# pengsongyou/openscene

Hardware: AMD Instinct MI355X
Metric: active voxels/sec MinkUNet18A fwd+bwd @2cm ScanNet; per-point query ms (higher is better)
Workload: dtype f32 (bf16x6 split-precision MFMA, fp32 accumulate); 1 GPU; ScanNet distillation step (configs[2]): MinkUNet18A, 768-d head, 1 synthetic S100k scene/GPU (100999 voxels on rank 0, 2 cm), training-mode BN; timed = coordinate+kernel maps, forward, cosine loss, backward, gradient all-reduce, Adam step; arch=MinkUNet18A, feature_dim=768, voxels_rank0=100999, parallelism=dp1

## Files before the change

### include/openscene_amd.h

```cpp
#ifndef OPENSCENE_AMD_H
#define OPENSCENE_AMD_H

#include <stddef.h>
#include <stdint.h>

#ifdef __cplusplus
extern "C" {
#endif

#define OSN_OK 0
#define OSN_E_ARG (-1)
#define OSN_E_HIP (-2)
#define OSN_E_WS (-3)
#define OSN_E_RANGE (-4)

typedef void* osn_stream_t;

int osn_version(void);
const char* osn_last_error(void);
int osn_device_ok(void);

int64_t osn_hash_capacity(int64_t n);
size_t osn_coords_unique_ws_bytes(int64_t n);

// ... 97 lines not shown
int osn_spconv_wgrad_plan(const int64_t* counts, int64_t n_out, int K, int cin, int cout,
                          int32_t* items , osn_stream_t stream);
int osn_spconv_wgrad(const float* in, const float* gout, const int32_t* nbr, const int64_t* counts,
                     const int32_t* plan_items, float* gW, int64_t n_out, int K, int cin, int cout,
                     void* ws, size_t ws_bytes, osn_stream_t stream);

size_t osn_pair_lists_bytes(int64_t n_out, int K, int bm);
int osn_pair_lists_build(const void* tl, const int32_t* out_rows, int64_t n_out, int K, int bm, void* pl,
                         osn_stream_t stream);
size_t osn_spconv_wgrad_tl_ws_bytes(int K, int cin, int cout);
int osn_spconv_wgrad_tl(const float* in, const float* gout, const void* pl, int swap, float* gW, int64_t n_in,
                        int64_t n_out, int K, int cin, int cout, void* ws, size_t ws_bytes, osn_stream_t stream);

typedef struct osn_wgrad_job {
    const float* partial;
    const void* range;
    float* gW;
    int32_t K, cin, cout, ident_items;
} osn_wgrad_job;
int osn_spconv_wgrad_tl_partial(const float* in, const float* gout, const void* pl, int swap, float* gW, int64_t n_in,
                                int64_t n_out, int K, int cin, int cout, void* partial, size_t partial_bytes,
                                osn_wgrad_job* job_host, osn_stream_t stream);
int osn_wgrad_tl_reduce_batch(const osn_wgrad_job* jobs_host, int n_jobs, osn_stream_t stream);

int osn_spconv_wgrad_tl_pieces(const float* in, const float* gout, const void* pl, int swap, float* gW, int64_t n_in,
                               int64_t n_out, int K, int cin, int cout, void* ws, size_t ws_bytes, osn_stream_t stream,
                               int pieces);
int osn_spconv_wgrad_tl_partial_pieces(const float* in, const float* gout, const void* pl, int swap, float* gW, int64_t n_in,
                                       int64_t n_out, int K, int cin, int cout, void* partial, size_t partial_bytes,
                                       osn_wgrad_job* job_host, osn_stream_t stream, int pieces);

int osn_dense_fwd(const float* in, const void* Wp, float* out, int64_t n, int cin, int cout, osn_stream_t stream);

int osn_spconv_fwd_rg_ok(int64_t n_in, int K, int cin, int cout);
int osn_spconv_fwd_rg(const float* in, int64_t n_in, const void* Wp, const int32_t* nbr, const int32_t* out_rows, float* out,
                      int64_t n_out, int K, int cin, int cout, osn_stream_t stream);

size_t osn_spconv_fwd_ws_ws_bytes(int64_t n_dst, int K, int cout, int direct);
int osn_spconv_fwd_ws(const float* in, int64_t n_in, const void* Wp, const void* pl, int64_t pl_rows, int swap, int direct,
                      const int32_t* nbr_dst, float* out, int64_t n_dst, int K, int cin, int cout, void* ws,
                      size_t ws_bytes, osn_stream_t stream);

int osn_stem_conv_fwd(const float* in, const float* W, const int32_t* nbr, float* out, int64_t n_out, int K,
                      int cin, int cout, osn_stream_t stream);
size_t osn_stem_conv_wgrad_ws_bytes(int K, int cin);
int osn_stem_conv_wgrad(const float* in, const float* gout, const int32_t* nbr, float* gW, int64_t n_out, int K, int cin,
// ... 381 lines not shown
```

### openscene_amd/_lib.py

```python
import ctypes
import os
import threading

_HERE = os.path.dirname(os.path.abspath(__file__))
LIB_PATH = os.environ.get("OSN_LIB_PATH") or os.path.join(_HERE, "lib", "libopenscene_amd.so")

_c = ctypes
_vp, _i32, _i64, _sz, _f32 = _c.c_void_p, _c.c_int, _c.c_int64, _c.c_size_t, _c.c_float

PROTOTYPES = {
    "osn_version": (_i32, []),
    "osn_last_error": (_c.c_char_p, []),
    "osn_device_ok": (_i32, []),
    "osn_hash_capacity": (_i64, [_i64]),
    "osn_coords_unique_ws_bytes": (_sz, [_i64]),
    "osn_coords_unique": (_i32, [_vp, _i64, _i32, _vp, _vp, _i64, _vp, _vp, _vp, _c.POINTER(_i64), _vp, _sz, _vp]),
    "osn_coords_unique_async": (_i32, [_vp, _i64, _vp, _i32, _vp, _vp, _i64, _vp, _vp, _vp, _vp, _vp, _vp, _sz, _vp]),
    "osn_coords_pyramid_async": (_i32, [_vp, _i64, _vp, _i32, _vp, _vp, _i64, _vp, _vp, _vp, _vp, _vp, _sz, _vp]),
    "osn_kmap_build": (_i32, [_vp, _vp, _i64, _vp, _i64, _i32, _i32, _vp, _vp, _vp]),
    "osn_kmap_build_self": (_i32, [_vp, _vp, _i64, _vp, _i64, _i32, _i32, _vp, _vp, _vp]),
    "osn_kmap_transpose": (_i32, [_vp, _i64, _i32, _i64, _vp, _vp]),
    "osn_kmap_sort_ws_bytes": (_sz, [_i64]),
    "osn_kmap_sort": (_i32, [_vp, _i64, _i32, _vp, _vp, _vp, _vp, _vp, _sz, _vp]),
    "osn_kmap_count": (_i32, [_vp, _i64, _i32, _vp, _vp]),
# ... 31 lines not shown
    "osn_spconv_wgrad_tl_ws_bytes": (_sz, [_i32, _i32, _i32]),
    "osn_spconv_wgrad_tl": (_i32, [_vp, _vp, _vp, _i32, _vp, _i64, _i64, _i32, _i32, _i32, _vp, _sz, _vp]),
    "osn_distill_loss_state_bytes": (_sz, [_i64, _i64]),
    "osn_distill_loss_fwd": (_i32, [_vp, _vp, _vp, _i64, _i64, _i32, _i32, _vp, _vp, _sz, _vp]),
    "osn_distill_loss_bwd": (_i32, [_vp, _vp, _vp, _i64, _i64, _i32, _i32, _vp, _vp, _vp, _sz, _vp]),
    "osn_rows_gather": (_i32, [_vp, _vp, _i64, _i32, _vp, _vp]),
    "osn_rows_scatter_zero": (_i32, [_vp, _vp, _i64, _i32, _vp, _vp]),
    "osn_distill_loss_check": (_i32, [_vp, _i64, _i64, _vp]),
    "osn_stem_conv_wgrad_ws_bytes": (_sz, [_i32, _i32]),
    "osn_stem_conv_wgrad": (_i32, [_vp, _vp, _vp, _vp, _i64, _i32, _i32, _i32, _vp, _sz, _vp]),
    "osn_dense_fwd": (_i32, [_vp, _vp, _vp, _i64, _i32, _i32, _vp]),
    "osn_rows_argmax": (_i32, [_vp, _i64, _i32, _vp, _i64, _i64, _vp, _vp]),
    "osn_adam_step": (_i32, [_vp, _vp, _vp, _vp, _i64, _i64, _f32, _f32, _f32, _f32, _f32, _vp]),
    "osn_sgd_step": (_i32, [_vp, _vp, _vp, _i64, _f32, _f32, _f32, _f32, _i32, _i32, _vp]),
    "osn_seg_loss_state_bytes": (_sz, [_i64, _i32]),
    "osn_seg_loss_fwd": (_i32, [_vp, _vp, _vp, _i64, _i64, _i32, _i64, _vp, _vp, _vp, _vp, _sz, _vp]),
    "osn_seg_loss_bwd": (_i32, [_vp, _vp, _vp, _i64, _i32, _i64, _vp, _vp, _sz, _vp]),
    "osn_seg_loss_check": (_i32, [_vp, _i64, _i64, _i32, _vp]),
    "osn_seg_vote": (_i32, [_vp, _vp, _i64, _i64, _i32, _vp, _vp]),
    "osn_spconv_fwd_ws_ws_bytes": (_sz, [_i64, _i32, _i32, _i32]),
    "osn_spconv_fwd_ws": (_i32, [_vp, _i64, _vp, _vp, _i64, _i32, _i32, _vp, _vp, _i64, _i32, _i32, _i32, _vp, _sz, _vp]),
    "osn_spconv_wgrad_tl_partial": (_i32, [_vp, _vp, _vp, _i32, _vp, _i64, _i64, _i32, _i32, _i32, _vp, _sz, _vp, _vp]),
    "osn_wgrad_tl_reduce_batch": (_i32, [_vp, _i32, _vp]),
    "osn_spconv_wgrad_tl_pieces": (_i32, [_vp, _vp, _vp, _i32, _vp, _i64, _i64, _i32, _i32, _i32, _vp, _sz, _vp, _i32]),
    "osn_spconv_wgrad_tl_partial_pieces": (_i32, [_vp, _vp, _vp, _i32, _vp, _i64, _i64, _i32, _i32, _i32, _vp, _sz, _vp, _vp, _i32]),
    "osn_stem_conv_fwd": (_i32, [_vp, _vp, _vp, _vp, _i64, _i32, _i32, _i32, _vp]),
    "osn_bn_ws_bytes": (_sz, [_i64, _i32]),
    "osn_bn_stats": (_i32, [_vp, _i64, _i32, _vp, _vp, _vp, _vp, _f32, _vp, _sz, _vp]),
    "osn_bn_apply": (_i32, [_vp, _vp, _vp, _vp, _vp, _f32, _vp, _i32, _vp, _vp, _i64, _i64, _i32, _vp]),
    "osn_spconv_fwd_rg_ok": (_i32, [_i64, _i32, _i32, _i32]),
    "osn_spconv_fwd_rg": (_i32, [_vp, _i64, _vp, _vp, _vp, _vp, _i64, _i32, _i32, _i32, _vp]),
    "osn_bn_forward_train": (_i32, [_vp, _i64, _i32, _vp, _vp, _f32, _vp, _i32, _f32, _vp, _vp, _vp, _vp, _vp, _vp, _i64, _vp, _sz, _vp]),
    "osn_bn_backward": (_i32, [_vp, _vp, _vp, _vp, _i32, _vp, _vp, _vp, _vp, _f32, _i32, _i32, _vp, _vp, _vp, _vp, _i64, _i32,
                               _vp, _sz, _vp]),
    "osn_bn_apply_plan": (_i32, [_i64, _i32, _c.POINTER(_i32), _c.POINTER(_i32)]),
    "osn_bn_set_flat_kernels": (_i32, [_i32]),
    "osn_bn_set_separate_finalize": (_i32, [_i32]),
    "osn_net_plan_query": (_i32, [_vp, _vp, _i32, _vp]),
    "osn_net_forward": (_i32, [_vp, _vp, _vp]),
    "osn_net_backward": (_i32, [_vp, _vp, _vp]),
    "osn_maps_build": (_i32, [_vp, _i32, _vp, _i32, _vp, _vp, _vp, _i32, _vp]),
    "osn_maps_occupancy_bytes": (_sz, [_i64]),
    "osn_maps_build_occ": (_i32, [_vp, _i32, _vp, _i32, _vp, _vp, _vp, _i32, _vp, _vp]),
    "osn_maps_set_legacy": (_i32, [_i32]),
    "osn_events_create": (_vp, [_i32]),
    "osn_events_destroy": (None, [_vp]),
# ... 139 lines not shown
```

### openscene_amd/csrc/pairlist.h

```cpp
#pragma once
#include "common.h"

namespace osn {

constexpr int PL_KMAX = 128;
constexpr int PL_ITEMS = 512;
constexpr int PL_MIN_QUOTA = 256;

constexpr size_t PL_OFF_POFF = 0;
constexpr size_t PL_OFF_TOTAL = 1024;
constexpr size_t PL_OFF_ITEMS = 2048;
constexpr size_t PL_OFF_RANGE = PL_OFF_ITEMS + size_t(PL_ITEMS) * 16;
constexpr size_t PL_OFF_PAIRS = 16384;

struct PlView {
    int32_t *poff, *total;
    int4* items;
    int2* range;
    int32_t *pin, *pout, *pref;
    size_t bytes;
};

static PlView pl_view(void* base, int64_t n_out, int K, int bm) {
    PlView v;
    char* p = static_cast<char*>(base);
    const size_t cap = size_t(K) * size_t(n_out > 0 ? n_out : 1);
    const size_t nt = size_t(cdiv(n_out > 0 ? n_out : 1, bm > 0 ? bm : 1));
    v.poff = reinterpret_cast<int32_t*>(p + PL_OFF_POFF);
    v.total = reinterpret_cast<int32_t*>(p + PL_OFF_TOTAL);
    v.items = reinterpret_cast<int4*>(p + PL_OFF_ITEMS);
// ... 10 lines not shown
```

### openscene_amd/csrc/wgrad_tl.hip

```cpp
#include "common.h"
#include "split.h"
#include <cstdlib>
#include "pairlist.h"
#include "coords_impl.h"

namespace osn {

typedef short s16x4 __attribute__((ext_vector_type(4)));

__device__ inline int wave_incl_scan_i32(int v, int lane) {
#pragma unroll
    for (int d = 1; d < 64; d <<= 1) {
        const int t = __shfl_up(v, d, 64);
        if (lane >= d) v += t;
    }
    return v;
}

__global__ __launch_bounds__(256) void pair_prefix_kernel(const int32_t* __restrict__ cnt, int n_tiles, int K,
                                                          int32_t* __restrict__ pref, int32_t* __restrict__ total) {
    __shared__ int wtot[4];
    __shared__ int carry_s;
    const int k = blockIdx.x, tid = threadIdx.x, lane = tid & 63, wave = tid >> 6;
    if (tid == 0) carry_s = 0;
// ... 83 lines not shown
    if (tid < K) range[tid] = make_int2(start[tid], start[tid + 1]);
    for (int t = tid; t < PL_ITEMS; t += 256) {
        int4 it = make_int4(-1, 0, 0, 0);
        if (t < start[K]) {
            int k = 0;
            while (k + 1 < K && start[k + 1] <= t) ++k;
            const int j = t - start[k];
            it.x = k;
            it.y = j * quota;
            it.z = min(it.y + quota, total[k]);
        }
        items[t] = it;
    }
}

__global__ __launch_bounds__(256) void pair_plan_kernel(const int32_t* __restrict__ total, int K, int4* __restrict__ items,
                                                        int2* __restrict__ range, int items_max) {
    pair_plan(total, K, items, range, items_max);
}

#define OSN_WG_TEMPLATE template <int MB, int NB, bool BUFG = false>
#define OSN_WG_NAME wgrad_tl_kernel
#define OSN_WG_NP 3
#include "wgrad_tl_kernel.h"
#undef OSN_WG_TEMPLATE
#undef OSN_WG_NAME
#undef OSN_WG_NP
#define OSN_WG_TEMPLATE template <int NP_, int MB, int NB, bool BUFG = false>
#define OSN_WG_NAME wgrad_tl_pieces_kernel
#define OSN_WG_NP NP_
#include "wgrad_tl_kernel.h"
#undef OSN_WG_TEMPLATE
#undef OSN_WG_NAME
#undef OSN_WG_NP

__global__ void wgrad_tl_reduce_kernel(const float* __restrict__ partial, const int2* __restrict__ range, int K, int cin,
                                       int cout, int transpose, int ident_items, float* __restrict__ out) {
    const int64_t per_k = int64_t(cin) * cout;
    const int64_t total = int64_t(K) * per_k;
    for (int64_t e = int64_t(blockIdx.x) * blockDim.x + threadIdx.x; e < total; e += int64_t(gridDim.x) * blockDim.x) {
        const int k = int(e / per_k);
        const int64_t r = e - int64_t(k) * per_k;
        int64_t src = r;
        if (transpose) {
            const int ci = int(r / cout), co = int(r - int64_t(ci) * cout);
            src = int64_t(co) * cin + ci;
        }
        const int t0 = range ? range[k].x : 0, t1 = range ? range[k].y : ident_items;
        float s = 0.f;
        for (int t = t0; t < t1; ++t) s += partial[int64_t(t) * per_k + src];
        out[e] = s;
    }
}

constexpr int WG_BATCH = 32;
struct WgJobs {
    osn_wgrad_job j[WG_BATCH];
};
// ... 51 lines not shown
        OSN_HIP(hipMemsetAsync(v.items, 0xFF, size_t(PL_ITEMS) * 16, st));
        OSN_HIP(hipMemsetAsync(v.range, 0, size_t(PL_KMAX) * 8, st));
        return OSN_OK;
    }
    OSN_REQUIRE(tl, OSN_E_ARG, "osn_pair_lists_build: null tile lists");
    const int64_t nt = cdiv(n_out, bm);
    const int32_t* cnt = static_cast<const int32_t*>(tl);
    const int2* lst = reinterpret_cast<const int2*>(static_cast<const char*>(tl) + align_up(size_t(nt) * K * 4, 256));
    hipLaunchKernelGGL(pair_prefix_kernel, dim3(K), dim3(256), 0, st, cnt, int(nt), K, v.pref, v.total);
    const int items_max = PL_ITEMS;
    const bool own_plan = maps_legacy();
    if (own_plan) hipLaunchKernelGGL(pair_plan_kernel, dim3(1), dim3(256), 0, st, v.total, K, v.items, v.range, items_max);
    hipLaunchKernelGGL(pair_fill_kernel, dim3(unsigned(nt)), dim3(256), 0, st, cnt, lst, out_rows, v.pref, v.total, int(nt), K,
                       bm, v.pin, v.pout, v.poff, own_plan ? nullptr : v.items, v.range, items_max);
    OSN_LAUNCH_CHECK();
    return OSN_OK;
}

namespace {
struct WgTlPlan {
    int mb, nb, n_ab, n_gb;
};
WgTlPlan plan_wg_tl(int ca, int cg) {
    auto blocks = [](int c) { int t = (c + 31) / 32; return t > 4 ? 4 : t; };
    WgTlPlan p;
    p.mb = blocks(ca);
    p.nb = blocks(cg);
    p.n_ab = int(cdiv(ca, 32 * p.mb));
    p.n_gb = int(cdiv(cg, 32 * p.nb));
    return p;
}
int ident_quota(int64_t n) {
    int64_t q = cdiv(n, PL_ITEMS);
    q = (q + 31) / 32 * 32;
    if (q < 64) q = 64;
    return int(q);
}
}

extern "C" size_t osn_spconv_wgrad_tl_ws_bytes(int K, int cin, int cout) {
    (void)K;
    return size_t(PL_ITEMS) * size_t(cin) * size_t(cout) * 4;
}

template <int MB>
static void launch_wg_tl_nb(int pieces, int nb, dim3 grid, hipStream_t st, const float* ra, const float* rg, const int32_t* ia,
                            const int32_t* ig, const int32_t* poff, const int4* items, float* partial, int ca, int cg,
                            int n_gb, int irows, int iquota, unsigned a_bytes, unsigned g_bytes) {
    const bool bufg = a_bytes != 0u && g_bytes != 0u;
#define OSN_WGTL_L(...)                                                                                                        \
    do {                                                                                                                       \
        if (bufg)                                                                                                              \
            hipLaunchKernelGGL((__VA_ARGS__, true>), grid, dim3(256), 0, st, ra, rg, ia, ig, poff, items, partial, ca, cg, n_gb, irows, \
                               iquota, a_bytes, g_bytes);                                                                      \
        else                                                                                                                   \
            hipLaunchKernelGGL((__VA_ARGS__, false>), grid, dim3(256), 0, st, ra, rg, ia, ig, poff, items, partial, ca, cg, n_gb, irows, \
                               iquota, 0u, 0u);                                                                                \
    } while (0)
#define OSN_WGTL(NB_)                                                                                                          \
    do {                                                                                                                       \
        if (pieces == 3) OSN_WGTL_L(wgrad_tl_kernel<MB, NB_);                                                                  \
        else if (pieces == 2) OSN_WGTL_L(wgrad_tl_pieces_kernel<2, MB, NB_);                                                   \
        else OSN_WGTL_L(wgrad_tl_pieces_kernel<1, MB, NB_);                                                                    \
    } while (0)
    switch (nb) {
        case 1: OSN_WGTL(1); break;
        case 2: OSN_WGTL(2); break;
        case 3: OSN_WGTL(3); break;
        default: OSN_WGTL(4); break;
    }
#undef OSN_WGTL
#undef OSN_WGTL_L
}

static int wgrad_tl_partial(const float* in, const float* gout, const void* pl, int swap, float* gW, int64_t n_in,
                            int64_t n_out, int K, int cin, int cout, void* ws, size_t ws_bytes, osn_wgrad_job* job,
                            int* launched, osn_stream_t stream, int pieces) {
    hipStream_t st = static_cast<hipStream_t>(stream);
    OSN_REQUIRE(pieces >= 1 && pieces <= 3, OSN_E_ARG, "osn_spconv_wgrad_tl: pieces=%d (1, 2 or 3)", pieces);
    OSN_REQUIRE(K >= 1 && K <= PL_KMAX && cin >= 4 && (cin & 3) == 0 && cout >= 4 && (cout & 3) == 0 && gW, OSN_E_ARG,
                "osn_spconv_wgrad_tl: needs cin %% 4 == 0 and cout %% 4 == 0 (K=%d cin=%d cout=%d)", K, cin, cout);
    OSN_REQUIRE(n_in >= 0 && n_out >= 0 && n_in < (int64_t(1) << 31) && n_out < (int64_t(1) << 31), OSN_E_ARG,
                "osn_spconv_wgrad_tl: row counts out of range");
    const int64_t wtotal = int64_t(K) * cin * cout;
    *launched = 0;
    if (n_out == 0 || n_in == 0) {
        OSN_HIP(hipMemsetAsync(gW, 0, size_t(wtotal) * 4, st));
        return OSN_OK;
    }
    OSN_REQUIRE(in && gout, OSN_E_ARG, "osn_spconv_wgrad_tl: null pointer");
    OSN_REQUIRE(pl || (K == 1 && n_in == n_out), OSN_E_ARG, "osn_spconv_wgrad_tl: pair lists may be null only for K == 1");
    OSN_REQUIRE(aligned16(in) && aligned16(gout) && aligned16(gW), OSN_E_ARG, "osn_spconv_wgrad_tl: pointers must be 16-byte aligned");
    const size_t need = osn_spconv_wgrad_tl_ws_bytes(K, cin, cout);
    OSN_REQUIRE(ws && ws_bytes >= need, OSN_E_WS, "osn_spconv_wgrad_tl: workspace %zu < %zu", ws_bytes, need);
    float* partial = static_cast<float*>(ws);
// ... 3 lines not shown
    const int32_t *ia = nullptr, *ig = nullptr, *poff = nullptr;
    const int4* items = nullptr;
    const int2* range = nullptr;
    int n_items = PL_ITEMS, irows = 0, iquota = 0;
    if (pl) {
        const int64_t table_rows = swap ? n_in : n_out;
        PlView v = pl_view(const_cast<void*>(pl), table_rows, K, 1);
        ia = swap ? v.pout : v.pin;
        ig = swap ? v.pin : v.pout;
        poff = v.poff;
        items = v.items;
        range = v.range;
    } else {
        irows = int(n_out);
        iquota = ident_quota(n_out);
        n_items = int(cdiv(n_out, iquota));
    }
    const WgTlPlan p = plan_wg_tl(ca, cg);
    const dim3 grid(unsigned(p.n_ab * p.n_gb), unsigned(n_items));
    const uint64_t ab64 = uint64_t(n_in) * uint64_t(cin) * 4u, gb64 = uint64_t(n_out) * uint64_t(cout) * 4u;
    const bool bufg = n_in < (int64_t(1) << 24) && n_out < (int64_t(1) << 24) && ab64 < (uint64_t(1) << 31) &&
                      gb64 < (uint64_t(1) << 31);
    const unsigned a_bytes = bufg ? unsigned(ab64) : 0u, g_bytes = bufg ? unsigned(gb64) : 0u;
    switch (p.mb) {
        case 1: launch_wg_tl_nb<1>(pieces, p.nb, grid, st, ra, rg, ia, ig, poff, items, partial, ca, cg, p.n_gb, irows, iquota, a_bytes, g_bytes); break;
        case 2: launch_wg_tl_nb<2>(pieces, p.nb, grid, st, ra, rg, ia, ig, poff, items, partial, ca, cg, p.n_gb, irows, iquota, a_bytes, g_bytes); break;
        case 3: launch_wg_tl_nb<3>(pieces, p.nb, grid, st, ra, rg, ia, ig, poff, items, partial, ca, cg, p.n_gb, irows, iquota, a_bytes, g_bytes); break;
        default: launch_wg_tl_nb<4>(pieces, p.nb, grid, st, ra, rg, ia, ig, poff, items, partial, ca, cg, p.n_gb, irows, iquota, a_bytes, g_bytes); break;
    }
    OSN_LAUNCH_CHECK();
    job->partial = partial;
    job->range = range;
    job->gW = gW;
    job->K = K; job->cin = cin; job->cout = cout; job->ident_items = n_items;
    *launched = 1;
    return OSN_OK;
}

static int wgrad_tl_whole(const float* in, const float* gout, const void* pl, int swap, float* gW, int64_t n_in, int64_t n_out, int K,
                          int cin, int cout, void* ws, size_t ws_bytes, osn_stream_t stream, int pieces) {
    hipStream_t st = static_cast<hipStream_t>(stream);
    osn_wgrad_job job;
    int launched = 0;
    int rc = wgrad_tl_partial(in, gout, pl, swap, gW, n_in, n_out, K, cin, cout, ws, ws_bytes, &job, &launched, stream, pieces);
    if (rc || !launched) return rc;
    const int64_t wtotal = int64_t(K) * cin * cout;
    int g = int(cdiv(wtotal, 256));
    if (g > 4096) g = 4096;
    hipLaunchKernelGGL(wgrad_tl_reduce_kernel, dim3(g), dim3(256), 0, st, job.partial, static_cast<const int2*>(job.range), K, cin,
                       cout, 0, job.ident_items, gW);
    OSN_LAUNCH_CHECK();
// ... 63 lines not shown
```

### openscene_amd/csrc/wgrad_tl_kernel.h

```cpp
OSN_WG_TEMPLATE
__global__ __launch_bounds__(256, 2) void OSN_WG_NAME(const float* __restrict__ rows_a, const float* __restrict__ rows_g,
                                                      const int32_t* __restrict__ idx_a, const int32_t* __restrict__ idx_g,
                                                      const int32_t* __restrict__ poff, const int4* __restrict__ items,
                                                      float* __restrict__ partial, int ca, int cg, int n_cgb,
                                                      int ident_rows, int ident_quota, unsigned a_bytes, unsigned g_bytes) {
    constexpr int NP = OSN_WG_NP;
    constexpr int CA_T = 32 * MB, CG_T = 32 * NB;
    constexpr int LDA = CA_T + 8, LDG = CG_T + 8;
    constexpr int QA = CA_T / 4, QG = CG_T / 4;
    __shared__ __attribute__((aligned(16))) __bf16 Ap[NP][32][LDA];
    __shared__ __attribute__((aligned(16))) __bf16 Gp[NP][32][LDG];
    __shared__ int idxbuf[2][32];

    const int tid = threadIdx.x, lane = tid & 63;
    const int wave = __builtin_amdgcn_readfirstlane(tid >> 6);
    const int wi = wave >> 1, wj = wave & 1;
    const int a0 = (blockIdx.x / n_cgb) * CA_T;
    const int g0 = (blockIdx.x % n_cgb) * CG_T;
    int k, p0, p1, base;
    int pstep = 32;
    if (idx_a) {
        const int4 it = items[blockIdx.y];
        k = it.x; p0 = it.y; p1 = it.z;
        if (k < 0) return;
        base = poff[k];
        const int n_it = it.w >> 16;
        if (n_it > 1) { p0 += 32 * (it.w & 0xFFFF); pstep = 32 * n_it; }
        if (p0 >= p1) p1 = p0;
    } else {
        k = 0; base = 0;
        p0 = blockIdx.y * ident_quota;
        p1 = min(p0 + ident_quota, ident_rows);
        if (p0 >= p1) return;
    }
    (void)k;

    f32x4 acc[MB][NB];
#pragma unroll
    for (int i = 0; i < MB; ++i)
#pragma unroll
        for (int j = 0; j < NB; ++j) acc[i][j] = f32x4{0.f, 0.f, 0.f, 0.f};

    int ar[MB], ac[MB], gr[NB], gc[NB];
#pragma unroll
    for (int j = 0; j < MB; ++j) { const int idx = tid + 256 * j; ar[j] = idx / QA; ac[j] = (idx - ar[j] * QA) * 4; }
#pragma unroll
    for (int j = 0; j < NB; ++j) { const int idx = tid + 256 * j; gr[j] = idx / QG; gc[j] = (idx - gr[j] * QG) * 4; }

    const __amdgpu_buffer_rsrc_t arsrc = __builtin_amdgcn_make_buffer_rsrc(const_cast<float*>(rows_a), 0, int(BUFG ? a_bytes : 0u), 0x00020000);
    const __amdgpu_buffer_rsrc_t grsrc = __builtin_amdgcn_make_buffer_rsrc(const_cast<float*>(rows_g), 0, int(BUFG ? g_bytes : 0u), 0x00020000);
    const unsigned ca4 = unsigned(ca) * 4u, cg4 = unsigned(cg) * 4u;
    float4 pa[MB], pg[NB];
    auto load_idx = [&](int p) -> int {
        const int q = p + (tid & 31);
        if (tid >= 64) return -1;
        if (q >= p1) return -1;
        if (!idx_a) return q;
        return tid < 32 ? idx_a[base + q] : idx_g[base + q];
    };
    auto fetch = [&](int par) {
#pragma unroll
        for (int j = 0; j < MB; ++j) {
            const int r = idxbuf[0][ar[j]];
            const int ch = a0 + ac[j];
            if constexpr (BUFG) {
                pa[j] = __builtin_bit_cast(float4, __builtin_amdgcn_raw_buffer_load_b128(
                                                       arsrc, __umul24(unsigned(max(r, 0)), ca4) + 4u * unsigned(ch), 0, 0));
                continue;
            }
            const bool ok = r >= 0 && ch < ca;
            const unsigned ru = ok ? unsigned(r) : 0u, cu = ok ? unsigned(ch) : 0u;
            pa[j] = *reinterpret_cast<const float4*>(rows_a + (uint64_t(ru) * unsigned(ca) + cu));
        }
#pragma unroll
        for (int j = 0; j < NB; ++j) {
            const int r = idxbuf[1][gr[j]];
            const int ch = g0 + gc[j];
            if constexpr (BUFG) {
                pg[j] = __builtin_bit_cast(float4, __builtin_amdgcn_raw_buffer_load_b128(
                                                       grsrc, __umul24(unsigned(max(r, 0)), cg4) + 4u * unsigned(ch), 0, 0));
                continue;
            }
            const bool ok = r >= 0 && ch < cg;
            const unsigned ru = ok ? unsigned(r) : 0u, cu = ok ? unsigned(ch) : 0u;
            pg[j] = *reinterpret_cast<const float4*>(rows_g + (uint64_t(ru) * unsigned(cg) + cu));
        }
        (void)par;
    };
    auto split4 = [&](const float4& v, bool ok, bf16x4& h1, bf16x4& h2, bf16x4& h3) {
        bf16x4 h[NP];
        tl_split4<NP>(ok ? v : make_float4(0.f, 0.f, 0.f, 0.f), h);
        h1 = h[0];
        if constexpr (NP > 1) h2 = h[1];
        if constexpr (NP > 2) h3 = h[2];
    };

    int ireg = load_idx(p0);
    if (tid < 64) idxbuf[tid >> 5][tid & 31] = ireg;
    __syncthreads();
    bool ok_a[MB], ok_g[NB];
    auto valid_now = [&]() {
#pragma unroll
        for (int j = 0; j < MB; ++j) ok_a[j] = idxbuf[0][ar[j]] >= 0 && a0 + ac[j] < ca;
#pragma unroll
        for (int j = 0; j < NB; ++j) ok_g[j] = idxbuf[1][gr[j]] >= 0 && g0 + gc[j] < cg;
    };
    valid_now();
    fetch(0);
    ireg = load_idx(p0 + pstep);

    for (int p = p0; p < p1; p += pstep) {
        bf16x4 a1[MB], a2[MB], a3[MB], g1[NB], g2[NB], g3[NB];
#pragma unroll
        for (int j = 0; j < MB; ++j) split4(pa[j], ok_a[j], a1[j], a2[j], a3[j]);
#pragma unroll
        for (int j = 0; j < NB; ++j) split4(pg[j], ok_g[j], g1[j], g2[j], g3[j]);
        __syncthreads();
#pragma unroll
        for (int j = 0; j < MB; ++j) {
            *reinterpret_cast<bf16x4*>(&Ap[0][ar[j]][ac[j]]) = a1[j];
            if constexpr (NP > 1) *reinterpret_cast<bf16x4*>(&Ap[1][ar[j]][ac[j]]) = a2[j];
            if constexpr (NP > 2) *reinterpret_cast<bf16x4*>(&Ap[2][ar[j]][ac[j]]) = a3[j];
        }
#pragma unroll
        for (int j = 0; j < NB; ++j) {
            *reinterpret_cast<bf16x4*>(&Gp[0][gr[j]][gc[j]]) = g1[j];
            if constexpr (NP > 1) *reinterpret_cast<bf16x4*>(&Gp[1][gr[j]][gc[j]]) = g2[j];
            if constexpr (NP > 2) *reinterpret_cast<bf16x4*>(&Gp[2][gr[j]][gc[j]]) = g3[j];
        }
        if (tid < 64) idxbuf[tid >> 5][tid & 31] = ireg;
        __syncthreads();
        if (p + pstep < p1) {
            valid_now();
            fetch(0);
            ireg = load_idx(p + 2 * pstep);
        }
        const int li = lane & 15, lg = lane >> 4;
        auto frag = [&](const __bf16* plane, int pitch, int c16) -> bf16x8 {
            const __bf16* q = plane + (8 * lg + (li >> 2)) * pitch + c16 + 4 * (li & 3);
            const s16x4 lo = __builtin_amdgcn_ds_read_tr16_b64_v4i16(
                (__attribute__((address_space(3))) s16x4*)(q));
            const s16x4 hi = __builtin_amdgcn_ds_read_tr16_b64_v4i16(
                (__attribute__((address_space(3))) s16x4*)(q + 4 * pitch));
            union { s16x4 h[2]; bf16x8 v; } u;
            u.h[0] = lo; u.h[1] = hi;
            return u.v;
        };
        bf16x8 fa[MB][NP], fg[NB][NP];
#pragma unroll
        for (int i = 0; i < MB; ++i)
#pragma unroll
            for (int pl = 0; pl < NP; ++pl) fa[i][pl] = frag(&Ap[pl][0][0], LDA, (wi * MB + i) * 16);
#pragma unroll
        for (int j = 0; j < NB; ++j)
#pragma unroll
            for (int pl = 0; pl < NP; ++pl) fg[j][pl] = frag(&Gp[pl][0][0], LDG, (wj * NB + j) * 16);
#pragma unroll
        for (int i = 0; i < MB; ++i)
#pragma unroll
            for (int j = 0; j < NB; ++j) {
                f32x4 t = acc[i][j];
                split_products<NP>([&](auto ap, auto gp) {
                    t = __builtin_amdgcn_mfma_f32_16x16x32_bf16(fa[i][ap], fg[j][gp], t, 0, 0, 0);
                });
                acc[i][j] = t;
            }
    }

    float* d = partial + int64_t(blockIdx.y) * ca * cg;
#pragma unroll
    for (int i = 0; i < MB; ++i)
#pragma unroll
        for (int j = 0; j < NB; ++j) {
            const int co = g0 + (wj * NB + j) * 16 + (lane & 15);
#pragma unroll
            for (int r = 0; r < 4; ++r) {
                const int ci = a0 + (wi * MB + i) * 16 + 4 * (lane >> 4) + r;
                if (ci < ca && co < cg) d[int64_t(ci) * cg + co] = acc[i][j][r];
            }
        }
}
```

### openscene_amd/ops.py

```python
import ctypes
import os
import threading
import weakref

import torch

from . import _lib
from ._lib import check

_vp = ctypes.c_void_p

_profiler = None


def set_profiler(p):
    global _profiler
    _profiler = p


_raw_stream_of = torch._C._cuda_getCurrentRawStream
_current_device = torch._C._cuda_getDevice


def _prof_start(kind, dev, **meta):
# ... 631 lines not shown
    if tl is not None:
        table_rows = n_in if swap else n_out
        if tl.K != K or tl.n_out != table_rows:
            raise ValueError("pair lists are for a [%d, %d] table, the weight gradient wants [%d, %d]" % (
                tl.K, tl.n_out, K, table_rows))
        pl = pair_lists(tl)
    else:
        if K != 1 or n_in != n_out:
            raise ValueError("tl=None is the identity map and needs K == 1 and n_in == n_out")
        pl = None
    gw = torch.empty((K, cin, cout), dtype=torch.float32, device=dev)
    wsb = _cached("osn_spconv_wgrad_tl_ws_bytes", K, cin, cout)
    ws = _ws(wsb, dev)
    tok = _prof_start("spconv_wgrad_tl", dev, n_in=n_in, n_out=n_out, K=K, cin=cin, cout=cout)
    with _Dev(dev):
        args = (_p(feats), _p(gout), _p(pl), int(bool(swap)), _p(gw), n_in, n_out, K, cin, cout, _p(ws), ws.numel(), _stream(dev))
        if pieces == 3:
            check(lib.osn_spconv_wgrad_tl(*args), "osn_spconv_wgrad_tl")
        else:
            check(lib.osn_spconv_wgrad_tl_pieces(*args, pieces), "osn_spconv_wgrad_tl_pieces")
    if tok is not None:
        _profiler.stop(tok)
    return gw


def rows_argmax(scores, gather=None):
    dev = scores.device
    lib = _prep(dev)
    if scores.dtype != torch.float32 or scores.dim() != 2 or scores.stride(1) != 1:
        raise ValueError("scores must be a float32 matrix with unit column stride")
    n, c = scores.shape
    ld = scores.stride(0) if n > 1 else max(c, scores.stride(0))
    if gather is not None:
        if gather.dtype != torch.int64 or gather.device != dev:
            raise ValueError("gather must be an int64 vector on the scores' device")
        gather = gather.contiguous()
    n_pts = n if gather is None else gather.shape[0]
    labels = torch.empty(n_pts, dtype=torch.int64, device=dev)
    with _Dev(dev):
        check(lib.osn_rows_argmax(_p(scores), ld, c, _p(gather), n_pts, n, _p(labels), _stream(dev)), "osn_rows_argmax")
    return labels


def dense_eligible(cin, cout):
    return bool(_cached("osn_dense_fwd_ok", int(cin), int(cout)))

# ... 1982 lines not shown
```

Before: 13.23 million voxels/s.

## Process multiple 32-pair sub-steps per iteration in narrow wgrad tiles

The weight-gradient pair-list kernel now stages several 32-pair sub-tiles (64 or 128 pairs) in LDS per loop iteration for narrow channel tiles (MB,NB<=2), picked by a constexpr table by tile shape and split pieces. Each barrier pair and index load then covers more MFMA work, which cuts sync overhead and exposes more memory-level parallelism for small-channel layers. It adds a runtime override (atomic global plus C API) that dispatches to extra template instantiations. The cost is higher LDS and register use, which can lower occupancy, and more padded work at segment tails.

Measured after the change: 13.23 million voxels/s (median of 3 runs). Within noise of the previous version (+0.0%).

```diff
diff --git a/include/openscene_amd.h b/include/openscene_amd.h
--- a/include/openscene_amd.h
+++ b/include/openscene_amd.h
@@ -143,6 +143,9 @@
                                 int64_t n_out, int K, int cin, int cout, void* partial, size_t partial_bytes,
                                 osn_wgrad_job* job_host, osn_stream_t stream);
 int osn_wgrad_tl_reduce_batch(const osn_wgrad_job* jobs_host, int n_jobs, osn_stream_t stream);
+
+int osn_spconv_wgrad_tl_step_pairs(int cin, int cout, int pieces);
+int osn_wgrad_tl_set_step_pairs(int pairs);
 
 int osn_spconv_wgrad_tl_pieces(const float* in, const float* gout, const void* pl, int swap, float* gW, int64_t n_in,
                                int64_t n_out, int K, int cin, int cout, void* ws, size_t ws_bytes, osn_stream_t stream,
diff --git a/openscene_amd/_lib.py b/openscene_amd/_lib.py
--- a/openscene_amd/_lib.py
+++ b/openscene_amd/_lib.py
@@ -77,6 +77,8 @@
     "osn_spconv_fwd_ws": (_i32, [_vp, _i64, _vp, _vp, _i64, _i32, _i32, _vp, _vp, _i64, _i32, _i32, _i32, _vp, _sz, _vp]),
     "osn_spconv_wgrad_tl_partial": (_i32, [_vp, _vp, _vp, _i32, _vp, _i64, _i64, _i32, _i32, _i32, _vp, _sz, _vp, _vp]),
     "osn_wgrad_tl_reduce_batch": (_i32, [_vp, _i32, _vp]),
+    "osn_spconv_wgrad_tl_step_pairs": (_i32, [_i32, _i32, _i32]),
+    "osn_wgrad_tl_set_step_pairs": (_i32, [_i32]),
     "osn_spconv_wgrad_tl_pieces": (_i32, [_vp, _vp, _vp, _i32, _vp, _i64, _i64, _i32, _i32, _i32, _vp, _sz, _vp, _i32]),
     "osn_spconv_wgrad_tl_partial_pieces": (_i32, [_vp, _vp, _vp, _i32, _vp, _i64, _i64, _i32, _i32, _i32, _vp, _sz, _vp, _vp, _i32]),
     "osn_stem_conv_fwd": (_i32, [_vp, _vp, _vp, _vp, _i64, _i32, _i32, _i32, _vp]),
diff --git a/openscene_amd/csrc/pairlist.h b/openscene_amd/csrc/pairlist.h
--- a/openscene_amd/csrc/pairlist.h
+++ b/openscene_amd/csrc/pairlist.h
@@ -6,6 +6,19 @@
 constexpr int PL_KMAX = 128;
 constexpr int PL_ITEMS = 512;
 constexpr int PL_MIN_QUOTA = 256;
+
+constexpr int tl_wg_blocks(int c) { return (c + 31) / 32 > 4 ? 4 : (c + 31) / 32; }
+constexpr int tl_step_lds(int mb, int nb, int np, int ps) { return np * ps * ((32 * mb + 8) + (32 * nb + 8)) * 2 + 8 * ps; }
+constexpr bool tl_step_narrow(int mb, int nb) { return mb <= 2 && nb <= 2; }
+constexpr int tl_step_pairs_blocks(int mb, int nb, int np) {
+    if (!tl_step_narrow(mb, nb)) return 32;
+    if (mb == 1 && nb == 1) return np == 3 ? 32 : 128;
+    if (mb == 1 && nb == 2) return 64;
+    if (mb == 2 && nb == 1) return np == 1 ? 32 : 64;
+    return 32;
+}
+static_assert(tl_step_lds(1, 1, 2, 128) <= 65536 && tl_step_lds(1, 2, 3, 64) <= 65536 && tl_step_lds(2, 1, 3, 64) <= 65536, "LDS budget");
+constexpr int tl_step_pairs(int cin, int cout, int pieces) { return tl_step_pairs_blocks(tl_wg_blocks(cin), tl_wg_blocks(cout), pieces); }
 
 constexpr size_t PL_OFF_POFF = 0;
 constexpr size_t PL_OFF_TOTAL = 1024;
diff --git a/openscene_amd/csrc/wgrad_tl.hip b/openscene_amd/csrc/wgrad_tl.hip
--- a/openscene_amd/csrc/wgrad_tl.hip
+++ b/openscene_amd/csrc/wgrad_tl.hip
@@ -1,5 +1,6 @@
 #include "common.h"
 #include "split.h"
+#include <atomic>
 #include <cstdlib>
 #include "pairlist.h"
 #include "coords_impl.h"
@@ -129,18 +130,21 @@
 #define OSN_WG_TEMPLATE template <int MB, int NB, bool BUFG = false>
 #define OSN_WG_NAME wgrad_tl_kernel
 #define OSN_WG_NP 3
+#define OSN_WG_PS tl_step_pairs_blocks(MB, NB, 3)
 #include "wgrad_tl_kernel.h"
 #undef OSN_WG_TEMPLATE
 #undef OSN_WG_NAME
 #undef OSN_WG_NP
-#define OSN_WG_TEMPLATE template <int NP_, int MB, int NB, bool BUFG = false>
+#undef OSN_WG_PS
+#define OSN_WG_TEMPLATE template <int NP_, int MB, int NB, bool BUFG = false, int PS_ = 0>
 #define OSN_WG_NAME wgrad_tl_pieces_kernel
 #define OSN_WG_NP NP_
+#define OSN_WG_PS (PS_ ? PS_ : tl_step_pairs_blocks(MB, NB, NP_))
 #include "wgrad_tl_kernel.h"
 #undef OSN_WG_TEMPLATE
 #undef OSN_WG_NAME
 #undef OSN_WG_NP
-
+#undef OSN_WG_PS
 __global__ void wgrad_tl_reduce_kernel(const float* __restrict__ partial, const int2* __restrict__ range, int K, int cin,
                                        int cout, int transpose, int ident_items, float* __restrict__ out) {
     const int64_t per_k = int64_t(cin) * cout;
@@ -238,10 +242,9 @@
     int mb, nb, n_ab, n_gb;
 };
 WgTlPlan plan_wg_tl(int ca, int cg) {
-    auto blocks = [](int c) { int t = (c + 31) / 32; return t > 4 ? 4 : t; };
     WgTlPlan p;
-    p.mb = blocks(ca);
-    p.nb = blocks(cg);
+    p.mb = tl_wg_blocks(ca);
+    p.nb = tl_wg_blocks(cg);
     p.n_ab = int(cdiv(ca, 32 * p.mb));
     p.n_gb = int(cdiv(cg, 32 * p.nb));
     return p;
@@ -259,34 +262,79 @@
     return size_t(PL_ITEMS) * size_t(cin) * size_t(cout) * 4;
 }
 
+static std::atomic<int> g_step_pairs{0};
+
+namespace {
+struct WgTlLaunch {
+    dim3 grid;
+    hipStream_t st;
+    const float *ra, *rg;
+    const int32_t *ia, *ig, *poff;
+    const int4* items;
+    float* partial;
+    int ca, cg, n_gb, irows, iquota;
+    unsigned a_bytes, g_bytes;
+};
+template <typename Kernel>
+void launch_wg_tl(Kernel kern, const WgTlLaunch& a) {
+    hipLaunchKernelGGL(kern, a.grid, dim3(256), 0, a.st, a.ra, a.rg, a.ia, a.ig, a.poff, a.items, a.partial, a.ca, a.cg, a.n_gb, a.irows,
+                       a.iquota, a.a_bytes, a.g_bytes);
+}
+template <int PS, int NP, int MB, int NB>
+void launch_wg_tl_step(bool bufg, const WgTlLaunch& a) {
+    if constexpr (tl_step_lds(MB, NB, NP, PS) <= 65536 && PS != tl_step_pairs_blocks(MB, NB, NP)) {
+        if (bufg) launch_wg_tl(wgrad_tl_pieces_kernel<NP, MB, NB, true, PS>, a);
+        else launch_wg_tl(wgrad_tl_pieces_kernel<NP, MB, NB, false, PS>, a);
+    }
+}
+template <int NP, int MB, int NB>
+void launch_wg_tl_inst(const WgTlLaunch& a) {
+    const bool bufg = a.a_bytes != 0u && a.g_bytes != 0u;
+    if constexpr (tl_step_narrow(MB, NB)) {
+        int want = g_step_pairs.load(std::memory_order_relaxed);
+        while (want > 32 && tl_step_lds(MB, NB, NP, want) > 65536) want /= 2;
+        if (want != 0 && want != tl_step_pairs_blocks(MB, NB, NP)) {
+            if (want == 128) launch_wg_tl_step<128, NP, MB, NB>(bufg, a);
+            else if (want == 64) launch_wg_tl_step<64, NP, MB, NB>(bufg, a);
+            else launch_wg_tl_step<32, NP, MB, NB>(bufg, a);
+            return;
+        }
+    }
+    if constexpr (NP == 3) {
+        if (bufg) launch_wg_tl(wgrad_tl_kernel<MB, NB, true>, a);
+        else launch_wg_tl(wgrad_tl_kernel<MB, NB, false>, a);
+    } else {
+        if (bufg) launch_wg_tl(wgrad_tl_pieces_kernel<NP, MB, NB, true>, a);
+        else launch_wg_tl(wgrad_tl_pieces_kernel<NP, MB, NB, false>, a);
+    }
+}
+template <int MB, int NB>
+void launch_wg_tl_np(int pieces, const WgTlLaunch& a) {
+    if (pieces == 3) launch_wg_tl_inst<3, MB, NB>(a);
+    else if (pieces == 2) launch_wg_tl_inst<2, MB, NB>(a);
+    else launch_wg_tl_inst<1, MB, NB>(a);
+}
 template <int MB>
-static void launch_wg_tl_nb(int pieces, int nb, dim3 grid, hipStream_t st, const float* ra, const float* rg, const int32_t* ia,
-                            const int32_t* ig, const int32_t* poff, const int4* items, float* partial, int ca, int cg,
-                            int n_gb, int irows, int iquota, unsigned a_bytes, unsigned g_bytes) {
-    const bool bufg = a_bytes != 0u && g_bytes != 0u;
-#define OSN_WGTL_L(...)                                                                                                        \
-    do {                                                                                                                       \
-        if (bufg)                                                                                                              \
-            hipLaunchKernelGGL((__VA_ARGS__, true>), grid, dim3(256), 0, st, ra, rg, ia, ig, poff, items, partial, ca, cg, n_gb, irows, \
-                               iquota, a_bytes, g_bytes);                                                                      \
-        else                                                                                                                   \
-            hipLaunchKernelGGL((__VA_ARGS__, false>), grid, dim3(256), 0, st, ra, rg, ia, ig, poff, items, partial, ca, cg, n_gb, irows, \
-                               iquota, 0u, 0u);                                                                                \
-    } while (0)
-#define OSN_WGTL(NB_)                                                                                                          \
-    do {                                                                                                                       \
-        if (pieces == 3) OSN_WGTL_L(wgrad_tl_kernel<MB, NB_);                                                                  \
-        else if (pieces == 2) OSN_WGTL_L(wgrad_tl_pieces_kernel<2, MB, NB_);                                                   \
-        else OSN_WGTL_L(wgrad_tl_pieces_kernel<1, MB, NB_);                                                                    \
-    } while (0)
+void launch_wg_tl_nb(int pieces, int nb, const WgTlLaunch& a) {
     switch (nb) {
-        case 1: OSN_WGTL(1); break;
-        case 2: OSN_WGTL(2); break;
-        case 3: OSN_WGTL(3); break;
-        default: OSN_WGTL(4); break;
-    }
-#undef OSN_WGTL
-#undef OSN_WGTL_L
+        case 1: launch_wg_tl_np<MB, 1>(pieces, a); break;
+        case 2: launch_wg_tl_np<MB, 2>(pieces, a); break;
+        case 3: launch_wg_tl_np<MB, 3>(pieces, a); break;
+        default: launch_wg_tl_np<MB, 4>(pieces, a); break;
+    }
+}
+}
+
+extern "C" int osn_spconv_wgrad_tl_step_pairs(int cin, int cout, int pieces) {
+    OSN_REQUIRE(cin >= 1 && cout >= 1 && pieces >= 1 && pieces <= 3, OSN_E_ARG, "osn_spconv_wgrad_tl_step_pairs: cin=%d cout=%d pieces=%d",
+                cin, cout, pieces);
+    return tl_step_pairs(cin, cout, pieces);
+}
+
+extern "C" int osn_wgrad_tl_set_step_pairs(int pairs) {
+    OSN_REQUIRE(pairs == 0 || pairs == 32 || pairs == 64 || pairs == 128, OSN_E_ARG, "osn_wgrad_tl_set_step_pairs: %d (0, 32, 64 or 128)",
+                pairs);
+    return g_step_pairs.exchange(pairs);
 }
 
 static int wgrad_tl_partial(const float* in, const float* gout, const void* pl, int swap, float* gW, int64_t n_in,
@@ -336,11 +384,12 @@
     const bool bufg = n_in < (int64_t(1) << 24) && n_out < (int64_t(1) << 24) && ab64 < (uint64_t(1) << 31) &&
                       gb64 < (uint64_t(1) << 31);
     const unsigned a_bytes = bufg ? unsigned(ab64) : 0u, g_bytes = bufg ? unsigned(gb64) : 0u;
+    const WgTlLaunch la{grid, st, ra, rg, ia, ig, poff, items, partial, ca, cg, p.n_gb, irows, iquota, a_bytes, g_bytes};
     switch (p.mb) {
-        case 1: launch_wg_tl_nb<1>(pieces, p.nb, grid, st, ra, rg, ia, ig, poff, items, partial, ca, cg, p.n_gb, irows, iquota, a_bytes, g_bytes); break;
-        case 2: launch_wg_tl_nb<2>(pieces, p.nb, grid, st, ra, rg, ia, ig, poff, items, partial, ca, cg, p.n_gb, irows, iquota, a_bytes, g_bytes); break;
-        case 3: launch_wg_tl_nb<3>(pieces, p.nb, grid, st, ra, rg, ia, ig, poff, items, partial, ca, cg, p.n_gb, irows, iquota, a_bytes, g_bytes); break;
-        default: launch_wg_tl_nb<4>(pieces, p.nb, grid, st, ra, rg, ia, ig, poff, items, partial, ca, cg, p.n_gb, irows, iquota, a_bytes, g_bytes); break;
+        case 1: launch_wg_tl_nb<1>(pieces, p.nb, la); break;
+        case 2: launch_wg_tl_nb<2>(pieces, p.nb, la); break;
+        case 3: launch_wg_tl_nb<3>(pieces, p.nb, la); break;
+        default: launch_wg_tl_nb<4>(pieces, p.nb, la); break;
     }
     OSN_LAUNCH_CHECK();
     job->partial = partial;
diff --git a/openscene_amd/csrc/wgrad_tl_kernel.h b/openscene_amd/csrc/wgrad_tl_kernel.h
--- a/openscene_amd/csrc/wgrad_tl_kernel.h
+++ b/openscene_amd/csrc/wgrad_tl_kernel.h
@@ -8,9 +8,14 @@
     constexpr int CA_T = 32 * MB, CG_T = 32 * NB;
     constexpr int LDA = CA_T + 8, LDG = CG_T + 8;
     constexpr int QA = CA_T / 4, QG = CG_T / 4;
-    __shared__ __attribute__((aligned(16))) __bf16 Ap[NP][32][LDA];
-    __shared__ __attribute__((aligned(16))) __bf16 Gp[NP][32][LDG];
-    __shared__ int idxbuf[2][32];
+    constexpr int PS = OSN_WG_PS, NS = PS / 32;
+    static_assert(PS == 32 || PS == 64 || PS == 128, "pairs per step");
+    static_assert(tl_step_lds(MB, NB, NP, PS) <= 65536, "two workgroups per CU");
+    struct __attribute__((aligned(16))) StageA { __bf16 Ap[NP][32][LDA]; };
+    struct __attribute__((aligned(16))) StageG { __bf16 Gp[NP][32][LDG]; };
+    __shared__ StageA sa[NS];
+    __shared__ StageG sg[NS];
+    __shared__ int idxbuf[2][PS];
 
     const int tid = threadIdx.x, lane = tid & 63;
     const int wave = __builtin_amdgcn_readfirstlane(tid >> 6);
@@ -50,40 +55,47 @@
     const __amdgpu_buffer_rsrc_t arsrc = __builtin_amdgcn_make_buffer_rsrc(const_cast<float*>(rows_a), 0, int(BUFG ? a_bytes : 0u), 0x00020000);
     const __amdgpu_buffer_rsrc_t grsrc = __builtin_amdgcn_make_buffer_rsrc(const_cast<float*>(rows_g), 0, int(BUFG ? g_bytes : 0u), 0x00020000);
     const unsigned ca4 = unsigned(ca) * 4u, cg4 = unsigned(cg) * 4u;
-    float4 pa[MB], pg[NB];
+    float4 pa[NS][MB], pg[NS][NB];
+    const int isub = NS == 1 ? 0 : tid >> 6, ihalf = NS == 1 ? tid >> 5 : (tid >> 5) & 1;
     auto load_idx = [&](int p) -> int {
-        const int q = p + (tid & 31);
-        if (tid >= 64) return -1;
+        const int q = p + isub * pstep + (tid & 31);
+        if (tid >= 64 * NS) return -1;
         if (q >= p1) return -1;
         if (!idx_a) return q;
-        return tid < 32 ? idx_a[base + q] : idx_g[base + q];
+        return (NS == 1 ? tid < 32 : ihalf == 0) ? idx_a[base + q] : idx_g[base + q];
+    };
+    auto store_idx = [&](int v) {
+        if (tid < 64 * NS) idxbuf[ihalf][32 * isub + (tid & 31)] = v;
     };
     auto fetch = [&](int par) {
 #pragma unroll
-        for (int j = 0; j < MB; ++j) {
-            const int r = idxbuf[0][ar[j]];
-            const int ch = a0 + ac[j];
-            if constexpr (BUFG) {
-                pa[j] = __builtin_bit_cast(float4, __builtin_amdgcn_raw_buffer_load_b128(
-                                                       arsrc, __umul24(unsigned(max(r, 0)), ca4) + 4u * unsigned(ch), 0, 0));
-                continue;
-            }
-            const bool ok = r >= 0 && ch < ca;
-            const unsigned ru = ok ? unsigned(r) : 0u, cu = ok ? unsigned(ch) : 0u;
-            pa[j] = *reinterpret_cast<const float4*>(rows_a + (uint64_t(ru) * unsigned(ca) + cu));
-        }
-#pragma unroll
-        for (int j = 0; j < NB; ++j) {
-            const int r = idxbuf[1][gr[j]];
-            const int ch = g0 + gc[j];
-            if constexpr (BUFG) {
-                pg[j] = __builtin_bit_cast(float4, __builtin_amdgcn_raw_buffer_load_b128(
-                                                       grsrc, __umul24(unsigned(max(r, 0)), cg4) + 4u * unsigned(ch), 0, 0));
-                continue;
-            }
-            const bool ok = r >= 0 && ch < cg;
-            const unsigned ru = ok ? unsigned(r) : 0u, cu = ok ? unsigned(ch) : 0u;
-            pg[j] = *reinterpret_cast<const float4*>(rows_g + (uint64_t(ru) * unsigned(cg) + cu));
+        for (int s = 0; s < NS; ++s) {
+#pragma unroll
+            for (int j = 0; j < MB; ++j) {
+                const int r = idxbuf[0][32 * s + ar[j]];
+                const int ch = a0 + ac[j];
+                if constexpr (BUFG) {
+                    pa[s][j] = __builtin_bit_cast(float4, __builtin_amdgcn_raw_buffer_load_b128(
+                                                           arsrc, __umul24(unsigned(max(r, 0)), ca4) + 4u * unsigned(ch), 0, 0));
+                    continue;
+                }
+                const bool ok = r >= 0 && ch < ca;
+                const unsigned ru = ok ? unsigned(r) : 0u, cu = ok ? unsigned(ch) : 0u;
+                pa[s][j] = *reinterpret_cast<const float4*>(rows_a + (uint64_t(ru) * unsigned(ca) + cu));
+            }
+#pragma unroll
+            for (int j = 0; j < NB; ++j) {
+                const int r = idxbuf[1][32 * s + gr[j]];
+                const int ch = g0 + gc[j];
+                if constexpr (BUFG) {
+                    pg[s][j] = __builtin_bit_cast(float4, __builtin_amdgcn_raw_buffer_load_b128(
+                                                           grsrc, __umul24(unsigned(max(r, 0)), cg4) + 4u * unsigned(ch), 0, 0));
+                    continue;
+                }
+                const bool ok = r >= 0 && ch < cg;
+                const unsigned ru = ok ? unsigned(r) : 0u, cu = ok ? unsigned(ch) : 0u;
+                pg[s][j] = *reinterpret_cast<const float4*>(rows_g + (uint64_t(ru) * unsigned(cg) + cu));
+            }
         }
         (void)par;
     };
@@ -95,45 +107,55 @@
         if constexpr (NP > 2) h3 = h[2];
     };
 
+    const int bstep = NS * pstep;
     int ireg = load_idx(p0);
-    if (tid < 64) idxbuf[tid >> 5][tid & 31] = ireg;
+    store_idx(ireg);
     __syncthreads();
-    bool ok_a[MB], ok_g[NB];
+    bool ok_a[NS][MB], ok_g[NS][NB];
     auto valid_now = [&]() {
 #pragma unroll
-        for (int j = 0; j < MB; ++j) ok_a[j] = idxbuf[0][ar[j]] >= 0 && a0 + ac[j] < ca;
-#pragma unroll
-        for (int j = 0; j < NB; ++j) ok_g[j] = idxbuf[1][gr[j]] >= 0 && g0 + gc[j] < cg;
+        for (int s = 0; s < NS; ++s) {
+#pragma unroll
+            for (int j = 0; j < MB; ++j) ok_a[s][j] = idxbuf[0][32 * s + ar[j]] >= 0 && a0 + ac[j] < ca;
+#pragma unroll
+            for (int j = 0; j < NB; ++j) ok_g[s][j] = idxbuf[1][32 * s + gr[j]] >= 0 && g0 + gc[j] < cg;
+        }
     };
     valid_now();
     fetch(0);
-    ireg = load_idx(p0 + pstep);
-
-    for (int p = p0; p < p1; p += pstep) {
-        bf16x4 a1[MB], a2[MB], a3[MB], g1[NB], g2[NB], g3[NB];
-#pragma unroll
-        for (int j = 0; j < MB; ++j) split4(pa[j], ok_a[j], a1[j], a2[j], a3[j]);
-#pragma unroll
-        for (int j = 0; j < NB; ++j) split4(pg[j], ok_g[j], g1[j], g2[j], g3[j]);
+    ireg = load_idx(p0 + bstep);
+
+    for (int p = p0; p < p1; p += bstep) {
+        bf16x4 a1[NS][MB], a2[NS][MB], a3[NS][MB], g1[NS][NB], g2[NS][NB], g3[NS][NB];
+#pragma unroll
+        for (int s = 0; s < NS; ++s) {
+#pragma unroll
+            for (int j = 0; j < MB; ++j) split4(pa[s][j], ok_a[s][j], a1[s][j], a2[s][j], a3[s][j]);
+#pragma unroll
+            for (int j = 0; j < NB; ++j) split4(pg[s][j], ok_g[s][j], g1[s][j], g2[s][j], g3[s][j]);
+        }
         __syncthreads();
 #pragma unroll
-        for (int j = 0; j < MB; ++j) {
-            *reinterpret_cast<bf16x4*>(&Ap[0][ar[j]][ac[j]]) = a1[j];
-            if constexpr (NP > 1) *reinterpret_cast<bf16x4*>(&Ap[1][ar[j]][ac[j]]) = a2[j];
-            if constexpr (NP > 2) *reinterpret_cast<bf16x4*>(&Ap[2][ar[j]][ac[j]]) = a3[j];
-        }
-#pragma unroll
-        for (int j = 0; j < NB; ++j) {
-            *reinterpret_cast<bf16x4*>(&Gp[0][gr[j]][gc[j]]) = g1[j];
-            if constexpr (NP > 1) *reinterpret_cast<bf16x4*>(&Gp[1][gr[j]][gc[j]]) = g2[j];
-            if constexpr (NP > 2) *reinterpret_cast<bf16x4*>(&Gp[2][gr[j]][gc[j]]) = g3[j];
-        }
-        if (tid < 64) idxbuf[tid >> 5][tid & 31] = ireg;
+        for (int s = 0; s < NS; ++s) {
+#pragma unroll
+            for (int j = 0; j < MB; ++j) {
+                *reinterpret_cast<bf16x4*>(&sa[s].Ap[0][ar[j]][ac[j]]) = a1[s][j];
+                if constexpr (NP > 1) *reinterpret_cast<bf16x4*>(&sa[s].Ap[1][ar[j]][ac[j]]) = a2[s][j];
+                if constexpr (NP > 2) *reinterpret_cast<bf16x4*>(&sa[s].Ap[2][ar[j]][ac[j]]) = a3[s][j];
+            }
+#pragma unroll
+            for (int j = 0; j < NB; ++j) {
+                *reinterpret_cast<bf16x4*>(&sg[s].Gp[0][gr[j]][gc[j]]) = g1[s][j];
+                if constexpr (NP > 1) *reinterpret_cast<bf16x4*>(&sg[s].Gp[1][gr[j]][gc[j]]) = g2[s][j];
+                if constexpr (NP > 2) *reinterpret_cast<bf16x4*>(&sg[s].Gp[2][gr[j]][gc[j]]) = g3[s][j];
+            }
+        }
+        store_idx(ireg);
         __syncthreads();
-        if (p + pstep < p1) {
+        if (p + bstep < p1) {
             valid_now();
             fetch(0);
-            ireg = load_idx(p + 2 * pstep);
+            ireg = load_idx(p + 2 * bstep);
         }
         const int li = lane & 15, lg = lane >> 4;
         auto frag = [&](const __bf16* plane, int pitch, int c16) -> bf16x8 {
@@ -146,25 +168,28 @@
             u.h[0] = lo; u.h[1] = hi;
             return u.v;
         };
-        bf16x8 fa[MB][NP], fg[NB][NP];
-#pragma unroll
-        for (int i = 0; i < MB; ++i)
-#pragma unroll
-            for (int pl = 0; pl < NP; ++pl) fa[i][pl] = frag(&Ap[pl][0][0], LDA, (wi * MB + i) * 16);
-#pragma unroll
-        for (int j = 0; j < NB; ++j)
-#pragma unroll
-            for (int pl = 0; pl < NP; ++pl) fg[j][pl] = frag(&Gp[pl][0][0], LDG, (wj * NB + j) * 16);
-#pragma unroll
-        for (int i = 0; i < MB; ++i)
-#pragma unroll
-            for (int j = 0; j < NB; ++j) {
-                f32x4 t = acc[i][j];
-                split_products<NP>([&](auto ap, auto gp) {
-                    t = __builtin_amdgcn_mfma_f32_16x16x32_bf16(fa[i][ap], fg[j][gp], t, 0, 0, 0);
-                });
-                acc[i][j] = t;
-            }
+#pragma unroll
+        for (int s = 0; s < NS; ++s) {
+            bf16x8 fa[MB][NP], fg[NB][NP];
+#pragma unroll
+            for (int i = 0; i < MB; ++i)
+#pragma unroll
+                for (int pl = 0; pl < NP; ++pl) fa[i][pl] = frag(&sa[s].Ap[pl][0][0], LDA, (wi * MB + i) * 16);
+#pragma unroll
+            for (int j = 0; j < NB; ++j)
+#pragma unroll
+                for (int pl = 0; pl < NP; ++pl) fg[j][pl] = frag(&sg[s].Gp[pl][0][0], LDG, (wj * NB + j) * 16);
+#pragma unroll
+            for (int i = 0; i < MB; ++i)
+#pragma unroll
+                for (int j = 0; j < NB; ++j) {
+                    f32x4 t = acc[i][j];
+                    split_products<NP>([&](auto ap, auto gp) {
+                        t = __builtin_amdgcn_mfma_f32_16x16x32_bf16(fa[i][ap], fg[j][gp], t, 0, 0, 0);
+                    });
+                    acc[i][j] = t;
+                }
+        }
     }
 
     float* d = partial + int64_t(blockIdx.y) * ca * cg;
diff --git a/openscene_amd/ops.py b/openscene_amd/ops.py
--- a/openscene_amd/ops.py
+++ b/openscene_amd/ops.py
@@ -677,6 +677,18 @@
     if tok is not None:
         _profiler.stop(tok)
     return gw
+
+
+def wgrad_tl_step_pairs(cin, cout, pieces=3):
+    ps = int(_lib.load().osn_spconv_wgrad_tl_step_pairs(int(cin), int(cout), int(pieces)))
+    check(min(ps, 0), "osn_spconv_wgrad_tl_step_pairs")
+    return ps
+
+
+def wgrad_tl_set_step_pairs(pairs):
+    prev = int(_lib.load().osn_wgrad_tl_set_step_pairs(int(pairs)))
+    check(min(prev, 0), "osn_wgrad_tl_set_step_pairs")
+    return prev
 
 
 def rows_argmax(scores, gather=None):
```
